# carlobaldassi/gimp-lqr-plugin

Measured on AMD Instinct MI355X. Metric: Mseams*pixels/sec on 4K RGBA, higher is better.
Workload: dtype f32; 1 GPU; batch4k: 64 x 3840x2160 RGBA per GPU, resize to 3640x2160 (200 vertical seams each), side-switch 2; images_per_gpu=64, width=3840, height=2160, new_width=3640, new_height=2160, parallelism=images sharded i mod N, no data-path collective, streams_per_gpu=1

## Files before the change

gimp-lqr-plugin_amd/csrc/lqr_shim.hip:

```cpp
#include "lqr_common.h"
#include "lqr_kernels.h"
#include "lqr_own.h"
#include <memory>

static thread_local std::string g_err;
static int g_device = -1;

static int *g_dev_err_host = nullptr;
static int *g_dev_err = nullptr;

#define HIPCK_VOID(expr) do { hipError_t e__ = (expr); if (e__ != hipSuccess) { g_err = std::string(#expr) + ": " + hipGetErrorString(e__); (void) hipGetLastError(); } } while (0)
#define HIPCK(expr)                                                                   \
    do {                                                                              \
        hipError_t e__ = (expr);                                                      \
        if (e__ != hipSuccess) {                                                      \
            g_err = std::string(#expr) + ": " + hipGetErrorString(e__);               \
            (void) hipGetLastError();                                                 \
            return (e__ == hipErrorOutOfMemory) ? LQRHIP_ENOMEM : LQRHIP_EHIP;        \
        }                                                                             \
    } while (0)

static PlanKnobs g_knobs;
static PlanDevice g_dev;

// ... 9 lines not shown
struct __attribute__((visibility("hidden"))) LqrHipCarver {
    int ch = 0;
    int depth = 0;
    int luma = 0;
    int mode = RD_RGB, alpha = -1, black = -1;
    int pix_deep = 0;
    int w0 = 0, h0 = 0;
    DevBuf<uint8_t> rgb0;
    DevBuf<int32_t> vs;
    DevBuf<float> bias0, rig0;
    int active = 0;
    int stride = 0, wk_h = 0;
    WorkingPlanes wk;
    int log_cap = 0, log_h = 0;
    int frozen_epoch = 0;
    LqrHipCarver *root = nullptr;
    std::vector<LqrHipCarver *> aux;
    LqrHipBatch *batch = nullptr;
};

static inline size_t px_bytes(const LqrHipCarver *c) { return (size_t) c->ch << (c->depth == 0 ? 0 : c->depth == 1 ? 1 : c->depth == 2 ? 2 : 3); }
static inline int32_t *vs_of(const LqrHipCarver *c) { return (c->root ? c->root : c)->vs; }

namespace {
struct PlaneJob {
    LqrHipCarver *c;
    DevBuf<uint8_t> nrgb;
    DevBuf<float> nbias, nrig;
};
}
// ... 27 lines not shown
};
static void commit(PlaneJobs &pj)
{
    for (auto &j : pj.jobs) {
        j.c->rgb0 = std::move(j.nrgb);
        if (j.nbias) j.c->bias0 = std::move(j.nbias);
        if (j.nrig) j.c->rig0 = std::move(j.nrig);
    }
}

struct PendingInflate { PlaneJobs pj; int kind = 0 , w1 = 0, h1 = 0; };

struct LqrHipBatch {
    std::vector<LqrHipCarver *> cs;
    DevCarver *d_desc = nullptr;
    hipStream_t stream = nullptr;
    DevBuf<unsigned long long> exch;
    int exch_ntiles = 0, exch_n = 0, exch_px = 0;
    int tile_epoch = 0;
    bool dirty = true;
    int shared_n = 1;
    bool shared = false;
    bool safe = false;
    std::unique_ptr<PendingInflate> pending_inflate;
};
static bool g_no_spin = false;

struct ProfRec {
    std::vector<std::pair<hipEvent_t, hipEvent_t>> ev;
    double bytes = 0;
// ... 429 lines not shown
    c->luma = luma != 0;
    return changed;
}

extern "C" int lqrhip_carver_set_read(LqrHipCarver *c, int image_type, int alpha, int black)
{
    static const int mode_of[8] = {RD_RGB, RD_RGB, RD_GREY, RD_GREY, RD_CMY, RD_CMYK, RD_CMYK, RD_CUSTOM};
    if (image_type < 0 || image_type > 7 || alpha >= c->ch || black >= c->ch) return LQRHIP_EARG;
    const bool was = reads_value(c);
    const int mode = mode_of[image_type], a = alpha < 0 ? -1 : alpha, k = black < 0 ? -1 : black;
    const bool differs = mode != c->mode || a != c->alpha || k != c->black;
    c->mode = mode; c->alpha = a; c->black = k;
    return (differs && (was || reads_value(c))) ? 1 : 0;
}

static void free_working(LqrHipCarver *c)
{
    c->wk = WorkingPlanes();
    c->log_cap = 0; c->log_h = 0;
}

extern "C" void lqrhip_carver_destroy(LqrHipCarver *c)
{
    if (!c) return;
    {
        LqrHipCarver *r = c->root ? c->root : c;
        if (r->batch && r->batch->stream) (void) hipStreamSynchronize(r->batch->stream);
        if (c->batch && c->batch != r->batch && c->batch->stream) (void) hipStreamSynchronize(c->batch->stream);
        if (g_stream0) (void) hipStreamSynchronize(g_stream0);
        (void) hipGetLastError();
    }
    delete c;
}

// ... 191 lines not shown
    tmp.done();
    return 0;
}

extern "C" void lqrhip_set_sub_batches(int n) { g_knobs.sub_batches = n > 0 ? n : 0; }
extern "C" int lqrhip_sub_batches(int n)
{
    const char *q = getenv("GPU_MAX_HW_QUEUES");
    g_dev.hw_queues = q ? atoi(q) : 0;
    return plan_streams(g_knobs, g_dev, n);
}

extern "C" void lqrhip_batch_set_shared(LqrHipBatch *b, int shared) { b->shared = shared != 0; b->shared_n = shared > 1 ? shared : 1; }
extern "C" void lqrhip_batch_set_safe(LqrHipBatch *b, int safe) { b->safe = safe != 0; if (safe) g_fault_stats[6]++; }

extern "C" LqrHipBatch *lqrhip_batch_create(LqrHipCarver **carvers, int n)
{
    if (lqrhip_init() < 0 || n <= 0) return nullptr;
    LqrHipBatch *b = new LqrHipBatch();
    for (int i = 0; i < n; i++) {
        b->cs.push_back(carvers[i]);
        carvers[i]->batch = b;
    }
    if (hipStreamCreateWithFlags(&b->stream, hipStreamNonBlocking) != hipSuccess ||
        hipMalloc((void **) &b->d_desc, sizeof(DevCarver) * n) != hipSuccess) {
        g_err = "batch_create failed";
        if (b->stream) (void) hipStreamDestroy(b->stream);
        for (auto *c : b->cs) if (c->batch == b) c->batch = nullptr;
        delete b;
        return nullptr;
    }
    g_live_batches.push_back(b);
    return b;
}

static void invalidate_all_batches(void)
{
    for (auto *b : g_live_batches) { b->exch_ntiles = 0; b->dirty = true; }
}

extern "C" void lqrhip_batch_abort(LqrHipBatch *b)
{
    if (!b) return;
    (void) hipStreamSynchronize(b->stream);
    (void) hipGetLastError();
    b->pending_inflate.reset();
    if (g_dev_err_host) *g_dev_err_host = 0;
    invalidate_all_batches();
}

extern "C" void lqrhip_batch_destroy(LqrHipBatch *b)
{
    if (!b) return;
    g_live_batches.erase(std::remove(g_live_batches.begin(), g_live_batches.end(), b), g_live_batches.end());
    if (b->stream) { (void) hipStreamSynchronize(b->stream); (void) hipStreamDestroy(b->stream); }
    for (auto *c : b->cs) if (c->batch == b) c->batch = nullptr;
    if (b->d_desc) (void) hipFree(b->d_desc);
    delete b;
}

extern "C" int lqrhip_batch_sync(LqrHipBatch *b)
{
    HIPCK(hipStreamSynchronize(b->stream));
    return check_dev_error();
}
extern "C" void *lqrhip_batch_stream(LqrHipBatch *b) { return (void *) b->stream; }

static DevCarver make_desc(const LqrHipCarver *c)
{
    DevCarver d;
    const WorkingPlanes &k = c->wk;
    d.rgb0 = c->rgb0; d.vs = vs_of(c); d.bias0 = c->bias0; d.rig0 = c->rig0;
// ... 75 lines not shown
    for (auto &e : it->second.ev) {
        float a = 0, b = 0;
        if (hipEventElapsedTime(&a, base, e.first) != hipSuccess) { (void) hipGetLastError(); float t = 0; if (hipEventElapsedTime(&t, e.first, base) == hipSuccess) a = -t; else (void) hipGetLastError(); }
        if (hipEventElapsedTime(&b, base, e.second) != hipSuccess) { (void) hipGetLastError(); float t = 0; if (hipEventElapsedTime(&t, e.second, base) == hipSuccess) b = -t; else (void) hipGetLastError(); }
        iv.emplace_back(a, b);
    }
    std::sort(iv.begin(), iv.end());
    float end = -1e30f;
    for (auto &p : iv) {
        if (p.first > end) { *ms_union += p.second - p.first; end = p.second; }
        else if (p.second > end) { *ms_union += p.second - end; end = p.second; }
    }
    return 0;
}

extern "C" int lqrhip_wk_init(LqrHipBatch *b, int from_visible)
{
    LqrHipCarver *c0 = b->cs[0];
    int w = c0->w0, h = c0->h0, rc;
    for (auto *c : b->cs) {
        if (c->w0 != w || c->h0 != h || c->ch != c0->ch || c->depth != c0->depth || c->luma != c0->luma || c->mode != c0->mode ||
            c->alpha != c0->alpha || c->black != c0->black)
            return LQRHIP_EARG;
        if ((rc = ensure_working(c, w, h))) return rc;
    }
    if ((rc = batch_upload(b))) return rc;
    for (auto *c : b->cs) c->frozen_epoch = 0;
    const dim3 grid((c0->stride + 255) / 256, h, (unsigned) b->cs.size()), grid_v(h, (unsigned) b->cs.size());
#define LAUNCH_WK(FORM, arg) do { if (from_visible) hipLaunchKernelGGL(k_wk_init_visible<FORM>, grid_v, dim3(256), 0, b->stream, b->d_desc, w, h, c0->stride, arg); \
                                  else hipLaunchKernelGGL(k_wk_init<FORM>, grid, dim3(256), 0, b->stream, b->d_desc, w, h, c0->stride, arg); } while (0)
    if (!reads_value(c0)) LAUNCH_WK(PixPacked, c0->ch);
    else if (c0->depth == 0) LAUNCH_WK(PixValue<0>, deep_read(c0));
    else if (c0->depth == 1) LAUNCH_WK(PixValue<1>, deep_read(c0));
    else if (c0->depth == 2) LAUNCH_WK(PixValue<2>, deep_read(c0));
    else LAUNCH_WK(PixValue<3>, deep_read(c0));
#undef LAUNCH_WK
    HIPCK(hipGetLastError());
    return 0;
}

extern "C" int lqrhip_emap_build(LqrHipBatch *b, const LqrHipDpParams *p, int w, int h)
{
    int rc;
    if ((rc = batch_upload(b))) return rc;
    LqrHipCarver *c0 = b->cs[0];
    dim3 grid((w + 255) / 256, h, (unsigned) b->cs.size());
    DpK k = make_dpk(p, c0->ch);
    const bool value = reads_value(c0);
    const int nrg = plane_nrg(value, nrg_index(p->nrg_func));
#define CASE(N, V) if (nrg == N && value == V) hipLaunchKernelGGL((k_emap_full<N, V>), grid, dim3(256), 0, b->stream, b->d_desc, k, w, h, c0->stride); else
    K_EMAP_FORMS(CASE) return no_form("k_emap_full");
#undef CASE
    HIPCK(hipGetLastError());
    return 0;
}

extern "C" int lqrhip_energy_out(LqrHipBatch *b, int w, int h, int transposed, int form, int depth, int image_type, void *out, int on_device)
{
// ... 187 lines not shown
{
    LqrHipCarver *c0 = b->cs[0];
    const int from = c0->frozen_epoch;
    if (to <= from) return 0;
    const int w_from = w_at_to + (to - from);
    size_t lds = (size_t) (to - from) * sizeof(int) + (size_t) w_from + 16;
    with_form(c0, [&](auto value) {
        hipLaunchKernelGGL(k_frozen_catchup<value>, dim3(h, (unsigned) b->cs.size()), dim3(256), lds, b->stream, b->d_desc, from, to, w_from, h,
                           c0->stride);
    });
    HIPCK(hipGetLastError());
    for (auto *c : b->cs) c->frozen_epoch = to;
    return 0;
}

static int launch_band_levels(LqrHipBatch *b, const DpK &k, int w, int h, int lr, int P, bool rigm)
{
    LqrHipCarver *c0 = b->cs[0];
    const size_t n = b->cs.size();
    int rc;
    const int ntiles = (w + 63) / 64;
    const size_t need_elems = 2 * ((size_t) 4 * LV_PMAX + (size_t) 2 * ntiles * 64) * n;
    if ((rc = exch_ensure(b, need_elems, ntiles, (int) n, 103))) return rc;
    const int epoch = 1 + ((b->tile_epoch++) % ((1 << 22) - 2));
    const dim3 grid((unsigned) (8 * ((n + 7) / 8) * P));
    CENSUS(LQRHIP_CENSUS_BAND_LEVELS);
    const DpForm f = dp_form(k, lr, rigm);
#define CASE(LR, RIG, DELTA, RIGM) if (f.lr == LR && f.rig == RIG && f.delta == DELTA && f.rigm == RIGM) \
        hipLaunchKernelGGL((k_band_levels<LR, RIG, DELTA, RIGM>), grid, dim3(128), 0, b->stream, b->d_desc, k, w, h, c0->stride, b->exch.get(), epoch, g_dev_err, P, (int) n); else
    K_BAND_LEVELS_FORMS(CASE) return no_form("k_band_levels");
// ... 28 lines not shown
        if (FILE *f = fopen(path, "wb")) {
            fwrite(hdr.data(), sizeof(int), hdr.size(), f); fwrite(flags.data(), sizeof(int), flags.size(), f);
            fwrite(seam.data(), sizeof(int), seam.size(), f); fwrite(m.data(), sizeof(float), np, f); fwrite(least.data(), 1, np, f);
            fclose(f);
        }
    }
    return rc;
}

static int seam_step_impl(LqrHipBatch *b, const LqrHipDpParams *p, int w, int h, int log_index, int leftright_pick,
                          int full_rebuild, int leftright_next)
{
    int rc;
    LqrHipCarver *c0 = b->cs[0];
    for (auto *c : b->cs)
        if (log_index >= c->log_cap) return LQRHIP_EARG;
    if ((rc = batch_upload(b))) return rc;
    const unsigned n = (unsigned) b->cs.size();
    DpK k = make_dpk(p, c0->ch);
    const int stride = c0->stride;
    const int wnew = w - 1;
    const int move_dp = (wnew > 1 && !full_rebuild) ? 1 : 0;
    const PlanBatch pb = plan_batch(b);
    const StepPlan s = plan_seam_step(g_knobs, g_dev, pb, p->delta_x, p->use_rigidity != 0, w, h, full_rebuild != 0, log_index + 1 - c0->frozen_epoch);
    const bool rigm = pb.rigm(p->use_rigidity != 0);
    const int moved_unit = 2 * (4 + (move_dp ? 5 : 0) + (pb.rigmask ? 4 : 0));
    if (s.backtrack == LQRHIP_CENSUS_VP_PARALLEL) {
        const int nchunks = s.vp_chunks, R4 = (s.vp_rows + 3) / 4;
        const size_t need = (size_t) (nchunks + 1) * stride + 64, need_path = need * 4 * R4;
        bool grew = false;
        for (auto *c : b->cs) {
// ... 78 lines not shown
        ProfScope ps("band_update", b->stream, 0);
        CENSUS(LQRHIP_CENSUS_BAND_GENERIC);
        hipLaunchKernelGGL(k_band_update, dim3(n), dim3(64), 0, b->stream, b->d_desc, k, wnew, h, stride, leftright_next);
    }
    {
        ProfScope ps("dp_update", b->stream, 0);
        if ((rc = launch_dp<true>(b, k, s.dp, rigm, wnew, h, leftright_next))) return rc;
    }
    HIPCK(hipGetLastError());
    return 0;
}

extern "C" int lqrhip_seam_log_reserve(LqrHipBatch *b, int n_seams, int h)
{
    int rc;
    for (auto *c : b->cs) if ((rc = ensure_log(c, n_seams, h))) return rc;
    return 0;
}

extern "C" int lqrhip_vs_commit(LqrHipBatch *b, int w0, int h0, int wc0, int n_seams, int first_level, int finish)
{
    int rc;
    if ((rc = batch_upload(b))) return rc;
    size_t lds = ((size_t) n_seams + wc0) * sizeof(int);
    if (lds > 150 * 1024) { g_err = "vs_commit: session too large for LDS"; return LQRHIP_EARG; }
    if (lds_needs_attr(lds)) {
        HIPCK(hipFuncSetAttribute((const void *) k_vs_commit, hipFuncAttributeMaxDynamicSharedMemorySize, (int) lds));
        CENSUS(LQRHIP_CENSUS_LDS_ATTR_COMMIT);
    }
    hipLaunchKernelGGL(k_vs_commit, dim3(h0, (unsigned) b->cs.size()), dim3(256), lds, b->stream, b->d_desc, w0, h0, wc0, n_seams,
                       first_level, finish);
    HIPCK(hipGetLastError());
    inject_after_commit(b, w0, h0, first_level);
    if ((rc = frozen_catchup(b, n_seams, wc0 - n_seams, h0))) return rc;
    for (auto *c : b->cs) c->frozen_epoch = 0;
    return 0;
}

static int g_selfcheck = 1, g_recovery = 1;
extern "C" void lqrhip_set_selfcheck(int on) { g_selfcheck = on != 0; }
extern "C" void lqrhip_set_recovery(int on) { g_recovery = on != 0; }
extern "C" int lqrhip_get_recovery(void) { return g_recovery; }
extern "C" int lqrhip_session_check(LqrHipBatch *b, int h, int wc0, int n_seams, int delta_x)
{
    int rc;
    if (!g_selfcheck || n_seams < 1) return 0;
    if ((rc = batch_upload(b))) return rc;
    hipLaunchKernelGGL(k_seam_check, dim3((h + 255) / 256, (unsigned) b->cs.size()), dim3(256), 0, b->stream, b->d_desc, h, wc0, n_seams, delta_x, g_dev_err);
    HIPCK(hipGetLastError());
    return 0;
}
extern "C" int lqrhip_session_rollback(LqrHipBatch *b, int w0, int h0, int first_level, int finish)
{
    (void) hipStreamSynchronize(b->stream);
    b->pending_inflate.reset();
    (void) hipGetLastError();
    if (g_dev_err_host) *g_dev_err_host = 0;
    invalidate_all_batches();
    int rc;
    if ((rc = batch_upload(b))) return rc;
    const size_t n = (size_t) w0 * h0;
    hipLaunchKernelGGL(k_vs_rollback, dim3((unsigned) std::min<size_t>((n + 255) / 256, 4096), (unsigned) b->cs.size()), dim3(256), 0, b->stream, b->d_desc, n, first_level, finish ? w0 : 0);
    HIPCK(hipGetLastError());
    HIPCK(hipStreamSynchronize(b->stream));
    for (auto *c : b->cs) c->frozen_epoch = 0;
    g_fault_stats[4]++;
    return 0;
}
static int g_inject_kind = 0, g_inject_step = 0, g_inject_times = 0;
extern "C" void lqrhip_debug_inject(int kind, int at_step, int times) { g_inject_kind = kind; g_inject_step = at_step; g_inject_times = kind ? std::max(times, 1) : 0; }
static void inject_after_step(LqrHipBatch *b, int h, int log_index)
{
    if (g_inject_times <= 0 || log_index != g_inject_step) return;
    if (g_inject_kind == 1 || g_inject_kind == 2) { *g_dev_err_host = g_inject_kind == 1 ? DEVERR_TILE_TIMEOUT : DEVERR_BAND_PREDICTION; }
    else if (g_inject_kind == 3 || g_inject_kind == 4) hipLaunchKernelGGL(k_inject, dim3(1), dim3(64), 0, b->stream, b->d_desc, g_inject_kind - 3, h, 0, log_index, 0);
    else return;
    g_inject_times--; g_fault_stats[5]++;
}
static void inject_after_commit(LqrHipBatch *b, int w0, int h0, int first_level)
{
// ... 37 lines not shown
        hipLaunchKernelGGL(k_inflate<false>, dim3(h0, (unsigned) pj.n_narrow), dim3(256), lds, b->stream, pj.d_dev.get(), w0, w1, l, max_level, g_selfcheck ? g_dev_err : (int *) nullptr);
    if (pj.n_wide())
        hipLaunchKernelGGL(k_inflate<true>, dim3(h0, (unsigned) pj.n_wide()), dim3(256), lds, b->stream, pj.d_wide(), w0, w1, l, max_level, g_selfcheck ? g_dev_err : (int *) nullptr);
    HIPCK(hipGetLastError());
    HIPCK(hipStreamSynchronize(b->stream));
    if ((rc = check_dev_error())) return rc;
    return st.kept();
}
extern "C" int lqrhip_planes_commit(LqrHipBatch *b)
{
    PendingInflate *pi = b->pending_inflate.get();
    if (!pi) return LQRHIP_EARG;
    PlaneJobs &pj = pi->pj;
    commit(pj);
    for (auto &j : pj.jobs) { j.c->w0 = pi->w1; j.c->h0 = pi->h1; }
    if (pi->kind != 2) {
        size_t i = 0;
        for (auto *c : b->cs) c->vs = std::move(pj.new_vs[i++]);
    }
    b->dirty = true;
    b->pending_inflate.reset();
    return 0;
}
extern "C" int lqrhip_inflate_commit(LqrHipBatch *b) { return lqrhip_planes_commit(b); }

extern "C" int lqrhip_flatten(LqrHipBatch *b, int w0, int h0, int w, int level)
{
    int rc;
    Staging st(b, 1, w, h0);
    PlaneJobs &pj = st.jobs();
// ... 85 lines not shown
    HIPCK(hipMemsetAsync(dout, 0, sizeof(int), g_stream0));
    hipLaunchKernelGGL(k_mask_line_max, dim3(n_lines), dim3(256), 0, g_stream0, d, channels, width, a0, b0, line_len, direction, dout);
    HIPCK(hipGetLastError());
    HIPCK(hipMemcpyAsync(&result, dout, sizeof(int), hipMemcpyDeviceToHost, g_stream0));
    HIPCK(hipStreamSynchronize(g_stream0));
    tmp.done();
    return result;
}

extern "C" void lqrhip_pool_trim(void)
{
    (void) hipDeviceSynchronize();
    for (auto &kv : g_pool_free) { (void) hipFree(kv.second); g_pool_size.erase(kv.second); }
    g_pool_free.clear();
    g_pool_cached = 0;
}

extern "C" int lqrhip_device_sync(void)
{
    HIPCK(hipDeviceSynchronize());
    return check_dev_error();
}

extern "C" int lqrhip_read_vmap(LqrHipCarver *c, int w0, int h0, int w, int level, int depth, int *out)
{
    int rc = batch_sync_of(c);
    if (rc) return rc;
    size_t n = (size_t) w * h0;
    Scratch tmp(g_stream0);
    int32_t *d = tmp.get<int32_t>(n, "&d", rc);
// ... 23 lines not shown
        for (int y = 0; y < h; y++) memcpy(en + (size_t) y * w, t.data() + (size_t) y * c->stride + org, (size_t) w * sizeof(float));
    }
    if (m) {
        HIPCK(hipMemcpy(t.data(), c->wk.m, n * sizeof(float), hipMemcpyDeviceToHost));
        for (int y = 0; y < h; y++) memcpy(m + (size_t) y * w, t.data() + (size_t) y * c->stride + org, (size_t) w * sizeof(float));
    }
    if (least_dx) {
        HIPCK(hipMemcpy(tl.data(), c->wk.least, n, hipMemcpyDeviceToHost));
        for (int y = 0; y < h; y++)
            for (int x = 0; x < w; x++) least_dx[(size_t) y * w + x] = y == 0 ? 0 : (int) tl[(size_t) y * c->stride + org + x];
    }
    return 0;
}

__global__ __launch_bounds__(256) void k_copy16(const u32x4 *__restrict__ src, u32x4 *__restrict__ dst, size_t n16);
extern "C" int lqrhip_carver_reset(LqrHipCarver *c, const void *device_rgb, int w, int h)
{
    if (!c || c->root || !c->aux.empty() || w < 1 || h < 1) return LQRHIP_EARG;
    int rc = batch_sync_of(c);
    if (rc) return rc;
    const size_t n = (size_t) w * h;
    c->rgb0.reset(); c->vs.reset(); c->bias0.reset(); c->rig0.reset();
    if (c->wk.bias || c->wk.rig) { free_working(c); c->stride = 0; c->wk_h = 0; }
    c->w0 = w; c->h0 = h;
    c->frozen_epoch = 0;
    if ((rc = c->rgb0.alloc(n * px_bytes(c), "&c->rgb0")) || (rc = c->vs.alloc(n, "&c->vs"))) return rc;
    {
        const size_t bytes = n * px_bytes(c), n16 = bytes / 16;
        if (n16 && !(((uintptr_t) device_rgb | (uintptr_t) c->rgb0.get()) & 15)) {
            hipLaunchKernelGGL(k_copy16, dim3((unsigned) ((n16 + 255) / 256)), dim3(256), 0, g_stream0, (const u32x4 *) device_rgb, (u32x4 *) c->rgb0.get(), n16);
            HIPCK(hipGetLastError());
            if (bytes & 15) HIPCK(hipMemcpyAsync(c->rgb0 + n16 * 16, (const uint8_t *) device_rgb + n16 * 16, bytes & 15, hipMemcpyDeviceToDevice, g_stream0));
        } else {
            HIPCK(hipMemcpyAsync(c->rgb0, device_rgb, bytes, hipMemcpyDeviceToDevice, g_stream0));
        }
    }
    HIPCK(hipMemsetAsync(c->vs, 0, n * sizeof(int32_t), g_stream0));
    if (c->batch) c->batch->dirty = true;
    if (c->active && (rc = ensure_working(c, w, h))) return rc;
    return 0;
}

extern "C" int lqrhip_reset_sync(void)
{
    if (g_stream0) HIPCK(hipStreamSynchronize(g_stream0));
    return 0;
}

extern "C" int lqrhip_mem_info(unsigned long long *free_bytes, unsigned long long *total_bytes, unsigned long long *cached_bytes)
{
    if (lqrhip_init() < 0) return LQRHIP_EHIP;
    size_t f = 0, t = 0;
    HIPCK(hipMemGetInfo(&f, &t));
    if (free_bytes) *free_bytes = f;
    if (total_bytes) *total_bytes = t;
    if (cached_bytes) *cached_bytes = g_pool_cached;
    return 0;
}

__global__ __launch_bounds__(256) void k_copy16(const u32x4 *__restrict__ src, u32x4 *__restrict__ dst, size_t n16)
{
    const size_t i = (size_t) blockIdx.x * 256 + threadIdx.x;
    if (i < n16) __builtin_nontemporal_store(__builtin_nontemporal_load((const GLOBAL_AS u32x4 *) src + i), (GLOBAL_AS u32x4 *) dst + i);
}

extern "C" int lqrhip_copy_bandwidth(unsigned long long bytes, int iters, double *gbps)
{
    if (lqrhip_init() < 0) return LQRHIP_EHIP;
    if (iters < 1 || bytes < 4096) return LQRHIP_EARG;
    struct Event { hipEvent_t e = nullptr; ~Event() { if (e) (void) hipEventDestroy(e); } } e0, e1;
    int rc;
    Scratch tmp(g_stream0);
    uint8_t *a = tmp.get<uint8_t>(bytes, "&a", rc);
    if (rc) return rc;
    uint8_t *b = tmp.get<uint8_t>(bytes, "&b", rc);
    if (rc) return rc;
    float ms = 0;
    const size_t n16 = bytes / 16;
// ... 57 lines not shown
```

gimp-lqr-plugin_amd/host/lqr_carver.c:

```c
#include <stdlib.h>
#include <string.h>
#include <stdio.h>
#include <math.h>

#include "../../include/lqr.h"
#include "../../include/lqr_coldepth.h"
#include "../../include/lqr_imagetype.h"
#include "../../include/lqr_masks.h"
#include "../../include/lqr_energy.h"
#include "../../include/lqr_hip.h"
#include "lqr_mask_queue.h"

#define MAXI(a, b) ((a) > (b) ? (a) : (b))
#define MINI(a, b) ((a) < (b) ? (a) : (b))

struct _LqrProgress {
    gfloat update_step;
    LqrProgressFuncInit init;
    LqrProgressFuncUpdate update;
    LqrProgressFuncEnd end;
    gchar init_width_message[LQR_PROGRESS_MAX_MESSAGE_LENGTH];
    gchar end_width_message[LQR_PROGRESS_MAX_MESSAGE_LENGTH];
    gchar init_height_message[LQR_PROGRESS_MAX_MESSAGE_LENGTH];
    gchar end_height_message[LQR_PROGRESS_MAX_MESSAGE_LENGTH];
};

struct _LqrVMap {
    gint *buffer;
    gint width, height, depth, orientation;
// ... 655 lines not shown
        if (w_before - 1 > 1) {
            if (r0->lr_switch_frequency && ((l - r0->max_level + lr_switch_interval / 2) % lr_switch_interval) == 0) {
                for (i = 0; i < g->n; i++) g->r[i]->leftright ^= 1;
                full = 1;
            }
        } else {
            finish = 1;
        }
        HIP_ALL(g, lqrhip_seam_step(B, &p, w_before, r0->h, l - r0->max_level, lr_pick, full, r0->leftright));
        for (i = 0; i < g->n; i++) { g->r[i]->level++; g->r[i]->w--; }
    }

    if (g_debug_snapshot)
        for (i = 0; i < g->n; i++) LQR_CATCH(take_debug_snapshot(g->r[i]));

    HIP_ALL(g, lqrhip_session_check(B, r0->h, wc0, n_seams, r0->delta_x));
    HIP_ALL(g, lqrhip_batch_sync(B));
    HIP_ALL(g, lqrhip_vs_commit(B, r0->w0, r0->h0, wc0, n_seams, first_level, finish));
    HIP_ALL(g, lqrhip_inflate(B, r0->w0, r0->h0, depth - 1, r0->max_level));
    HIP_ALL(g, lqrhip_planes_commit(B));
    w1 = r0->w0 + (depth - 1) - r0->max_level + 1;
    FOR_TREE(g, i, r, {
        r->level = depth; r->max_level = depth;
        r->w0 = w1;
        set_width_one(r, r->w_start);
    });
    return LQR_OK;
}

static LqrRetVal session_run(Group *g, int depth, int redo, int *reported)
{
    LqrCarver *r0 = g->r[0];
    LqrHipDpParams p;
    int i;
    for (i = 0; i < g->n; i++) set_width_one(g->r[i], g->r[i]->w_start - g->r[i]->max_level + 1);
// ... 168 lines not shown
static LqrRetVal group_resize(LqrCarver **rs, int n, int w1, int h1)
{
    Group g;
    LqrRetVal ret = LQR_OK;
    int i;
    if (w1 < 1 || h1 < 1) return LQR_ERROR;
    for (i = 0; i < n; i++)
        if (rs[i]->root || !rs[i]->progress) return LQR_ERROR;
    for (i = 0; i < n; i++) LQR_CATCH(mask_queue_flush(rs[i]));
    for (i = 0; i < n; i++)
        if (frame_refused(rs[i], w1, 0) || frame_refused(rs[i], h1, 1)) {
            fprintf(stderr, "liblqr-hip: resize refused: a frame wider than %d px in the direction being carved is not supported\n",
                    LQRHIP_MAX_FRAME_WIDTH);
            return LQR_ERROR;
        }
    LQR_CATCH(group_open(&g, rs, n));
    if (rs[0]->resize_order == LQR_RES_ORDER_HOR) {
        if ((ret = group_resize_dir(&g, w1, 0)) == LQR_OK) ret = group_resize_dir(&g, h1, 1);
    } else {
        if ((ret = group_resize_dir(&g, h1, 1)) == LQR_OK) ret = group_resize_dir(&g, w1, 0);
    }
    if (ret == LQR_OK) {
        int k;
        for (k = 0; k < g.nb; k++) { LqrRetVal rk = hip_ret(lqrhip_batch_sync(g.b[k])); if (ret == LQR_OK) ret = rk; }
    }
    if (ret != LQR_OK) { int k; for (k = 0; k < g.nb; k++) lqrhip_batch_abort(g.b[k]); }
    FOR_TREE(&g, i, r, { r->ro_valid = 0; r->ro_line = 0; r->ro_x = 0; });
    group_close(&g);
    return ret;
}

LqrRetVal lqr_carver_resize(LqrCarver *r, gint w1, gint h1) { return group_resize(&r, 1, w1, h1); }

LqrRetVal lqrx_carver_resize_batch(LqrCarver **carvers, gint n, gint w1, gint h1)
{
    int i, same = 1;
    if (n < 1) return LQR_ERROR;
    for (i = 1; i < n; i++) same &= same_config(carvers[0], carvers[i]);
    if (same) {
        const LqrCarver *c = carvers[0];
        if (is_general(c)) {
            int wmax = c->w_start > c->h_start ? c->w_start : c->h_start, lim;
            if (w1 > wmax) wmax = w1;
// ... 102 lines not shown
LqrRetVal lqrx_carver_read_image_device(LqrCarver *r, void *device_ptr)
{
    HIP_CATCH(lqrhip_read_visible_device(r->dev, r->w0, r->h0, r->w, r->level, device_ptr));
    return LQR_OK;
}

LqrRetVal lqrx_vmap_to_rgba(LqrVMap *v, const gdouble col_start[3], const gdouble col_end[3], guchar *out_rgba)
{
    if (!v || !v->buffer || !out_rgba) return LQR_ERROR;
    HIP_CATCH(lqrhip_vmap_to_rgba(v->buffer, v->width, v->height, v->depth, col_start, col_end, out_rgba));
    return LQR_OK;
}

LqrRetVal lqrx_carver_reload_device_batch(LqrCarver **rs, gint n, void *const *device_rgb)
{
    int i, x;
    if (n < 1) return LQR_ERROR;
    for (i = 0; i < n; i++)
        if (!rs[i] || rs[i]->root || rs[i]->attached || !device_rgb[i]) return LQR_ERROR;
    for (i = 0; i < n; i++) {
        LqrCarver *r = rs[i];
        LqrVMapList *v, *vn;
        lqr_maskq_reset(&r->mq[0]); lqr_maskq_reset(&r->mq[1]);
        HIP_CATCH(lqrhip_carver_reset(r->dev, device_rgb[i], r->img_w, r->img_h));
        for (v = r->flushed_vs; v; v = vn) { vn = v->next; lqr_vmap_destroy(v->current); free(v); }
        r->flushed_vs = NULL;
        r->level = r->max_level = 1;
        r->w = r->w0 = r->w_start = r->img_w;
        r->h = r->h0 = r->h_start = r->img_h;
        r->transposed = 0;
        r->leftright = 0;
        r->has_bias = r->has_rigmask = 0;
        r->wk_valid = 0;
        r->ro_valid = 0; r->ro_line = 0; r->ro_x = 0;
        if (r->active)
            for (x = -r->delta_x; x <= r->delta_x; x++)
                r->rigidity_map[x + r->delta_x] = r->rigidity * powf(fabsf((float) x), 1.5f) / r->h;
    }
    HIP_CATCH(lqrhip_reset_sync());
    return LQR_OK;
}

gint lqrx_guess_new_size(const guchar *mask, gint channels, gint width, gint height, gint x_off, gint y_off,
                         gint old_width, gint old_height, gint direction)
{
    int lw = MINI(old_width, width + x_off) - MAXI(0, x_off);
    int lh = MINI(old_height, height + y_off) - MAXI(0, y_off);
    int old_size = direction ? old_height : old_width, m;
    if (direction == 0)
        m = lqrhip_mask_line_max(mask, channels, width, height, MAXI(0, y_off) - y_off, MAXI(0, -x_off),
                                 MINI(old_height, height + y_off) - MAXI(0, y_off), lw, 0);
    else
        m = lqrhip_mask_line_max(mask, channels, width, height, MAXI(0, x_off) - x_off, MAXI(0, -y_off),
                                 MINI(old_width, width + x_off) - MAXI(0, x_off), lh, 1);
// ... 82 lines not shown
```

include/lqr_hip.h:

```cpp
#ifndef LQR_HIP_H
#define LQR_HIP_H

#include <stddef.h>

#ifdef __cplusplus
extern "C" {
#endif

#define LQRHIP_OK 0
#define LQRHIP_ENOMEM (-2)
#define LQRHIP_EHIP (-1)
#define LQRHIP_EARG (-3)
#define LQRHIP_EFAULT (-4)
#define LQRHIP_MAX_DELTA 16
#define LQRHIP_MAX_CHANNELS 64
#define LQRHIP_MAX_FRAME_WIDTH 16384

typedef struct LqrHipCarver LqrHipCarver;
typedef struct LqrHipBatch LqrHipBatch;

typedef struct LqrHipDpParams {
    int delta_x;
    int use_rigidity;
    float rigidity_map[2 * LQRHIP_MAX_DELTA + 1];
    int nrg_func;
    int nrg_radius;
    int w_start;
} LqrHipDpParams;

int lqrhip_init(void);
const char *lqrhip_last_error(void);

LqrHipCarver *lqrhip_carver_create(const unsigned char *rgb, int w, int h, int channels);
LqrHipCarver *lqrhip_carver_create_ext(const void *rgb, int w, int h, int channels, int depth);
int lqrhip_carver_set_read_luma(LqrHipCarver *c, int luma);
int lqrhip_carver_set_read(LqrHipCarver *c, int image_type, int alpha, int black);
void lqrhip_carver_destroy(LqrHipCarver *c);
int lqrhip_carver_reset(LqrHipCarver *c, const void *device_rgb, int w, int h);
int lqrhip_reset_sync(void);
int lqrhip_carver_attach(LqrHipCarver *root, LqrHipCarver *aux);
int lqrhip_carver_activate(LqrHipCarver *c);

int lqrhip_mask_add(LqrHipCarver *c, const unsigned char *mask, int channels, int width, int height,
                    int x_off, int y_off, int transposed, int is_rigmask, int bias_factor);

int lqrhip_mask_add_f(LqrHipCarver *c, const void *mask, int depth, int on_device, int width, int height, int x_off, int y_off,
                      int transposed, int is_rigmask, int bias_factor);
int lqrhip_mask_plane_ensure(LqrHipCarver *c, int is_rigmask);
int lqrhip_mask_scatter(LqrHipCarver *c, int is_rigmask, const int *index, const double *value, const size_t *start, int buckets);
int lqrhip_mask_clear(LqrHipCarver *c, int is_rigmask);
int lqrhip_read_mask_plane(LqrHipCarver *c, int is_rigmask, int transposed, float *out);
unsigned long long lqrhip_debug_mask_flushes(void);

// ... 16 lines not shown
                     int leftright_pick, int full_rebuild, int leftright_next);
int lqrhip_seam_log_reserve(LqrHipBatch *b, int n_seams, int h);
int lqrhip_vs_commit(LqrHipBatch *b, int w0, int h0, int wc0, int n_seams, int first_level, int finish);
int lqrhip_session_check(LqrHipBatch *b, int h, int wc0, int n_seams, int delta_x);
void lqrhip_set_selfcheck(int on);
void lqrhip_set_recovery(int on);
int lqrhip_get_recovery(void);
int lqrhip_session_rollback(LqrHipBatch *b, int w0, int h0, int first_level, int finish);
void lqrhip_batch_set_safe(LqrHipBatch *b, int safe);
void lqrhip_set_no_spin(int on);
int lqrhip_get_no_spin(void);
int lqrhip_fault_stats(unsigned long long *out8, int reset);
void lqrhip_debug_inject(int kind, int at_step, int times);
void lqrhip_debug_fail_alloc(int nth);
unsigned long long lqrhip_debug_pool_live(void);
int lqrhip_inflate(LqrHipBatch *b, int w0, int h0, int l, int max_level);
int lqrhip_flatten(LqrHipBatch *b, int w0, int h0, int w, int level);
int lqrhip_transpose(LqrHipBatch *b, int w, int h);
int lqrhip_planes_commit(LqrHipBatch *b);
int lqrhip_inflate_commit(LqrHipBatch *b);

int lqrhip_read_visible(LqrHipCarver *c, int w0, int h0, int w, int level, unsigned char *out);
int lqrhip_mask_line_max(const unsigned char *mask, int channels, int width, int height, int a0, int b0, int n_lines, int line_len,
                         int direction);
int lqrhip_read_visible_device(LqrHipCarver *c, int w0, int h0, int w, int level, void *device_out);
int lqrhip_device_sync(void);
int lqrhip_mem_info(unsigned long long *free_bytes, unsigned long long *total_bytes, unsigned long long *cached_bytes);
int lqrhip_copy_bandwidth(unsigned long long bytes, int iters, double *gbps);
int lqrhip_vmap_to_rgba(const int *vmap, int w, int h, int depth, const double col_start[3], const double col_end[3],
                        unsigned char *out_rgba);
// ... 47 lines not shown
```

Baseline: 501,300 Mseams*px/s.

## Cut fixed per-call costs: park streams, batch resets, defer frozen catchup

Destroyed batches now park their streams and descriptor buffers in a small pool for reuse instead of recreating them with hipStreamCreate and hipMalloc. Carver resets for a batch of same-sized images are merged into one multi-job kernel that copies the RGB planes and zeroes the seam maps, replacing a memcpy and memset per image. The frozen-epoch catchup after vs_commit is deferred and paid lazily at the next emap build or log reserve, so it can be skipped when state is dropped anyway. Optional host timing instrumentation is added behind a compile flag. This adds state-tracking complexity around deferred catchup and pooled resources.

```diff
diff --git a/gimp-lqr-plugin_amd/csrc/lqr_shim.hip b/gimp-lqr-plugin_amd/csrc/lqr_shim.hip
--- a/gimp-lqr-plugin_amd/csrc/lqr_shim.hip
+++ b/gimp-lqr-plugin_amd/csrc/lqr_shim.hip
@@ -47,6 +47,7 @@
     WorkingPlanes wk;
     int log_cap = 0, log_h = 0;
     int frozen_epoch = 0;
+    int owed_to = 0, owed_w = 0, owed_h = 0;
     LqrHipCarver *root = nullptr;
     std::vector<LqrHipCarver *> aux;
     LqrHipBatch *batch = nullptr;
@@ -104,6 +105,7 @@
 struct LqrHipBatch {
     std::vector<LqrHipCarver *> cs;
     DevCarver *d_desc = nullptr;
+    size_t desc_cap = 0;
     hipStream_t stream = nullptr;
     DevBuf<unsigned long long> exch;
     int exch_ntiles = 0, exch_n = 0, exch_px = 0;
@@ -563,10 +565,17 @@
     return (differs && (was || reads_value(c))) ? 1 : 0;
 }
 
+static inline void drop_catchup(LqrHipCarver *c)
+{
+    c->owed_to = 0; c->owed_w = 0; c->owed_h = 0;
+    c->frozen_epoch = 0;
+}
+
 static void free_working(LqrHipCarver *c)
 {
     c->wk = WorkingPlanes();
     c->log_cap = 0; c->log_h = 0;
+    drop_catchup(c);
 }
 
 extern "C" void lqrhip_carver_destroy(LqrHipCarver *c)
@@ -788,6 +797,24 @@
 extern "C" void lqrhip_batch_set_shared(LqrHipBatch *b, int shared) { b->shared = shared != 0; b->shared_n = shared > 1 ? shared : 1; }
 extern "C" void lqrhip_batch_set_safe(LqrHipBatch *b, int safe) { b->safe = safe != 0; if (safe) g_fault_stats[6]++; }
 
+static const size_t MAX_PARKED = 4;
+static std::vector<hipStream_t> g_parked_streams;
+static unsigned long long g_fixed_stats[3];
+static std::multimap<size_t, DevCarver *> g_parked_desc;
+extern "C" void lqrhip_debug_fixedcost(unsigned long long out4[4], int reset)
+{
+    out4[0] = g_parked_streams.size();
+    for (int i = 0; i < 3; i++) out4[i + 1] = g_fixed_stats[i];
+    if (reset) memset(g_fixed_stats, 0, sizeof g_fixed_stats);
+}
+static void unpark_all(void)
+{
+    for (hipStream_t s : g_parked_streams) (void) hipStreamDestroy(s);
+    g_parked_streams.clear();
+    for (auto &kv : g_parked_desc) (void) hipFree(kv.second);
+    g_parked_desc.clear();
+}
+
 extern "C" LqrHipBatch *lqrhip_batch_create(LqrHipCarver **carvers, int n)
 {
     if (lqrhip_init() < 0 || n <= 0) return nullptr;
@@ -796,9 +823,17 @@
         b->cs.push_back(carvers[i]);
         carvers[i]->batch = b;
     }
-    if (hipStreamCreateWithFlags(&b->stream, hipStreamNonBlocking) != hipSuccess ||
-        hipMalloc((void **) &b->d_desc, sizeof(DevCarver) * n) != hipSuccess) {
+    hipError_t e = hipSuccess;
+    if (!g_parked_streams.empty()) { b->stream = g_parked_streams.back(); g_parked_streams.pop_back(); g_fixed_stats[0]++; }
+    else e = hipStreamCreateWithFlags(&b->stream, hipStreamNonBlocking);
+    if (e == hipSuccess) {
+        auto it = g_parked_desc.lower_bound((size_t) n);
+        if (it != g_parked_desc.end()) { b->d_desc = it->second; b->desc_cap = it->first; g_parked_desc.erase(it); }
+        else if ((e = hipMalloc((void **) &b->d_desc, sizeof(DevCarver) * n)) == hipSuccess) b->desc_cap = (size_t) n;
+    }
+    if (e != hipSuccess) {
         g_err = "batch_create failed";
+        (void) hipGetLastError();
         if (b->stream) (void) hipStreamDestroy(b->stream);
         for (auto *c : b->cs) if (c->batch == b) c->batch = nullptr;
         delete b;
@@ -827,9 +862,16 @@
 {
     if (!b) return;
     g_live_batches.erase(std::remove(g_live_batches.begin(), g_live_batches.end(), b), g_live_batches.end());
-    if (b->stream) { (void) hipStreamSynchronize(b->stream); (void) hipStreamDestroy(b->stream); }
+    if (b->stream) (void) hipStreamSynchronize(b->stream);
     for (auto *c : b->cs) if (c->batch == b) c->batch = nullptr;
-    if (b->d_desc) (void) hipFree(b->d_desc);
+    if (b->stream) {
+        if (g_parked_streams.size() < MAX_PARKED) g_parked_streams.push_back(b->stream);
+        else (void) hipStreamDestroy(b->stream);
+    }
+    if (b->d_desc) {
+        if (g_parked_desc.size() < MAX_PARKED) g_parked_desc.emplace(b->desc_cap, b->d_desc);
+        else (void) hipFree(b->d_desc);
+    }
     delete b;
 }
 
@@ -935,6 +977,7 @@
     return 0;
 }
 
+static int pay_catchup(LqrHipBatch *b);
 extern "C" int lqrhip_wk_init(LqrHipBatch *b, int from_visible)
 {
     LqrHipCarver *c0 = b->cs[0];
@@ -946,7 +989,7 @@
         if ((rc = ensure_working(c, w, h))) return rc;
     }
     if ((rc = batch_upload(b))) return rc;
-    for (auto *c : b->cs) c->frozen_epoch = 0;
+    for (auto *c : b->cs) drop_catchup(c);
     const dim3 grid((c0->stride + 255) / 256, h, (unsigned) b->cs.size()), grid_v(h, (unsigned) b->cs.size());
 #define LAUNCH_WK(FORM, arg) do { if (from_visible) hipLaunchKernelGGL(k_wk_init_visible<FORM>, grid_v, dim3(256), 0, b->stream, b->d_desc, w, h, c0->stride, arg); \
                                   else hipLaunchKernelGGL(k_wk_init<FORM>, grid, dim3(256), 0, b->stream, b->d_desc, w, h, c0->stride, arg); } while (0)
@@ -963,6 +1006,7 @@
 extern "C" int lqrhip_emap_build(LqrHipBatch *b, const LqrHipDpParams *p, int w, int h)
 {
     int rc;
+    if ((rc = pay_catchup(b))) return rc;
     if ((rc = batch_upload(b))) return rc;
     LqrHipCarver *c0 = b->cs[0];
     dim3 grid((w + 255) / 256, h, (unsigned) b->cs.size());
@@ -1180,6 +1224,36 @@
     return 0;
 }
 
+static int pay_catchup(LqrHipBatch *b)
+{
+    LqrHipCarver *c0 = b->cs[0];
+    bool any = false, alike = true;
+    for (auto *c : b->cs) {
+        any |= c->owed_to > 0;
+        alike &= c->owed_to == c0->owed_to && c->owed_w == c0->owed_w && c->owed_h == c0->owed_h && c->frozen_epoch == c0->frozen_epoch && c->stride == c0->stride;
+    }
+    if (!any) return 0;
+    int rc;
+    if ((rc = batch_upload(b))) return rc;
+    if (alike) {
+        if ((rc = frozen_catchup(b, c0->owed_to, c0->owed_w, c0->owed_h))) return rc;
+    } else {
+        for (size_t i = 0; i < b->cs.size(); i++) {
+            LqrHipCarver *c = b->cs[i];
+            if (c->owed_to <= c->frozen_epoch) continue;
+            const int from = c->frozen_epoch, w_from = c->owed_w + (c->owed_to - from);
+            const size_t lds = (size_t) (c->owed_to - from) * sizeof(int) + (size_t) w_from + 16;
+            with_form(c, [&](auto value) {
+                hipLaunchKernelGGL(k_frozen_catchup<value>, dim3(c->owed_h, 1), dim3(256), lds, b->stream, b->d_desc + i, from, c->owed_to, w_from, c->owed_h, c->stride);
+            });
+            HIPCK(hipGetLastError());
+            drop_catchup(c);
+        }
+    }
+    for (auto *c : b->cs) drop_catchup(c);
+    return 0;
+}
+
 static int launch_band_levels(LqrHipBatch *b, const DpK &k, int w, int h, int lr, int P, bool rigm)
 {
     LqrHipCarver *c0 = b->cs[0];
@@ -1238,7 +1312,7 @@
     int rc;
     LqrHipCarver *c0 = b->cs[0];
     for (auto *c : b->cs)
-        if (log_index >= c->log_cap) return LQRHIP_EARG;
+        if (log_index >= c->log_cap || c->owed_to) return LQRHIP_EARG;
     if ((rc = batch_upload(b))) return rc;
     const unsigned n = (unsigned) b->cs.size();
     DpK k = make_dpk(p, c0->ch);
@@ -1347,6 +1421,7 @@
 extern "C" int lqrhip_seam_log_reserve(LqrHipBatch *b, int n_seams, int h)
 {
     int rc;
+    if ((rc = pay_catchup(b))) return rc;
     for (auto *c : b->cs) if ((rc = ensure_log(c, n_seams, h))) return rc;
     return 0;
 }
@@ -1365,8 +1440,10 @@
                        first_level, finish);
     HIPCK(hipGetLastError());
     inject_after_commit(b, w0, h0, first_level);
-    if ((rc = frozen_catchup(b, n_seams, wc0 - n_seams, h0))) return rc;
-    for (auto *c : b->cs) c->frozen_epoch = 0;
+    for (auto *c : b->cs) {
+        if (c->frozen_epoch < n_seams) { c->owed_to = n_seams; c->owed_w = wc0 - n_seams; c->owed_h = h0; }
+        else drop_catchup(c);
+    }
     return 0;
 }
 
@@ -1396,7 +1473,7 @@
     hipLaunchKernelGGL(k_vs_rollback, dim3((unsigned) std::min<size_t>((n + 255) / 256, 4096), (unsigned) b->cs.size()), dim3(256), 0, b->stream, b->d_desc, n, first_level, finish ? w0 : 0);
     HIPCK(hipGetLastError());
     HIPCK(hipStreamSynchronize(b->stream));
-    for (auto *c : b->cs) c->frozen_epoch = 0;
+    for (auto *c : b->cs) drop_catchup(c);
     g_fault_stats[4]++;
     return 0;
 }
@@ -1464,6 +1541,8 @@
     PlaneJobs &pj = pi->pj;
     commit(pj);
     for (auto &j : pj.jobs) { j.c->w0 = pi->w1; j.c->h0 = pi->h1; }
+    if (pi->kind != 0)
+        for (auto *c : b->cs) drop_catchup(c);
     if (pi->kind != 2) {
         size_t i = 0;
         for (auto *c : b->cs) c->vs = std::move(pj.new_vs[i++]);
@@ -1579,6 +1658,7 @@
     for (auto &kv : g_pool_free) { (void) hipFree(kv.second); g_pool_size.erase(kv.second); }
     g_pool_free.clear();
     g_pool_cached = 0;
+    unpark_all();
 }
 
 extern "C" int lqrhip_device_sync(void)
@@ -1632,17 +1712,24 @@
 }
 
 __global__ __launch_bounds__(256) void k_copy16(const u32x4 *__restrict__ src, u32x4 *__restrict__ dst, size_t n16);
-extern "C" int lqrhip_carver_reset(LqrHipCarver *c, const void *device_rgb, int w, int h)
-{
-    if (!c || c->root || !c->aux.empty() || w < 1 || h < 1) return LQRHIP_EARG;
+static int reset_planes(LqrHipCarver *c, int w, int h)
+{
     int rc = batch_sync_of(c);
     if (rc) return rc;
     const size_t n = (size_t) w * h;
     c->rgb0.reset(); c->vs.reset(); c->bias0.reset(); c->rig0.reset();
     if (c->wk.bias || c->wk.rig) { free_working(c); c->stride = 0; c->wk_h = 0; }
     c->w0 = w; c->h0 = h;
-    c->frozen_epoch = 0;
+    drop_catchup(c);
     if ((rc = c->rgb0.alloc(n * px_bytes(c), "&c->rgb0")) || (rc = c->vs.alloc(n, "&c->vs"))) return rc;
+    return 0;
+}
+extern "C" int lqrhip_carver_reset(LqrHipCarver *c, const void *device_rgb, int w, int h)
+{
+    if (!c || c->root || !c->aux.empty() || w < 1 || h < 1) return LQRHIP_EARG;
+    int rc = reset_planes(c, w, h);
+    if (rc) return rc;
+    const size_t n = (size_t) w * h;
     {
         const size_t bytes = n * px_bytes(c), n16 = bytes / 16;
         if (n16 && !(((uintptr_t) device_rgb | (uintptr_t) c->rgb0.get()) & 15)) {
@@ -1659,6 +1746,56 @@
     return 0;
 }
 
+enum { RESET_JOBS = 16 };
+struct ResetJob { const uint8_t *src; uint8_t *dst; uint8_t *vs; size_t bytes; };
+struct ResetJobs { ResetJob j[RESET_JOBS]; };
+__global__ __launch_bounds__(256) void k_reset_jobs(const ResetJobs jobs, const size_t vs_bytes);
+static int g_reset_batch_count = 0;
+extern "C" int lqrhip_carver_reset_batch_count(void) { return g_reset_batch_count; }
+extern "C" int lqrhip_carver_reset_batch(LqrHipCarver **cs, const void *const *device_rgb, int n, int w, int h)
+{
+    g_reset_batch_count = 0;
+    if (!cs || !device_rgb || n < 1 || w < 1 || h < 1) return LQRHIP_EARG;
+    for (int i = 0; i < n; i++)
+        if (!cs[i] || cs[i]->root || !cs[i]->aux.empty() || !device_rgb[i]) return LQRHIP_EARG;
+    const size_t npx = (size_t) w * h, vs_bytes = npx * sizeof(int32_t);
+    ResetJobs jobs = {};
+    int nj = 0;
+    size_t most = vs_bytes;
+    auto flush = [&]() -> int {
+        if (!nj) return 0;
+        const unsigned blocks = (unsigned) std::min<size_t>((most / 16 + 255) / 256 + 1, 4096);
+        hipLaunchKernelGGL(k_reset_jobs, dim3(blocks, (unsigned) nj), dim3(256), 0, g_stream0, jobs, vs_bytes);
+        nj = 0; most = vs_bytes;
+        HIPCK(hipGetLastError());
+        return 0;
+    };
+    for (int i = 0; i < n; i++) {
+        LqrHipCarver *c = cs[i];
+        g_reset_batch_count = i;
+        int rc = reset_planes(c, w, h);
+        if (rc) { (void) flush(); return rc; }
+        const size_t bytes = npx * px_bytes(c);
+        if (!(((uintptr_t) device_rgb[i] | (uintptr_t) c->rgb0.get() | (uintptr_t) c->vs.get()) & 15)) {
+            jobs.j[nj++] = ResetJob{(const uint8_t *) device_rgb[i], c->rgb0.get(), (uint8_t *) c->vs.get(), bytes};
+            most = std::max(most, bytes);
+            g_fixed_stats[1]++;
+        } else {
+            g_fixed_stats[2]++;
+            hipError_t e = hipMemcpyAsync(c->rgb0, device_rgb[i], bytes, hipMemcpyDeviceToDevice, g_stream0);
+            if (e == hipSuccess) e = hipMemsetAsync(c->vs, 0, vs_bytes, g_stream0);
+            if (e != hipSuccess) { (void) flush(); HIPCK(e); }
+        }
+        if (c->batch) c->batch->dirty = true;
+        if (c->active && (rc = ensure_working(c, w, h))) { (void) flush(); return rc; }
+        if (nj == RESET_JOBS && (rc = flush())) return rc;
+    }
+    int rc = flush();
+    if (rc) return rc;
+    g_reset_batch_count = n;
+    return 0;
+}
+
 extern "C" int lqrhip_reset_sync(void)
 {
     if (g_stream0) HIPCK(hipStreamSynchronize(g_stream0));
@@ -1680,6 +1817,20 @@
 {
     const size_t i = (size_t) blockIdx.x * 256 + threadIdx.x;
     if (i < n16) __builtin_nontemporal_store(__builtin_nontemporal_load((const GLOBAL_AS u32x4 *) src + i), (GLOBAL_AS u32x4 *) dst + i);
+}
+
+__global__ __launch_bounds__(256) void k_reset_jobs(const ResetJobs jobs, const size_t vs_bytes)
+{
+    const ResetJob j = jobs.j[blockIdx.y];
+    const size_t tid = (size_t) blockIdx.x * 256 + threadIdx.x, nthreads = (size_t) gridDim.x * 256;
+    const size_t n16 = j.bytes / 16, z16 = vs_bytes / 16;
+    for (size_t i = tid; i < n16; i += nthreads)
+        __builtin_nontemporal_store(__builtin_nontemporal_load((const GLOBAL_AS u32x4 *) j.src + i), (GLOBAL_AS u32x4 *) j.dst + i);
+    const u32x4 zero = {0u, 0u, 0u, 0u};
+    for (size_t i = tid; i < z16; i += nthreads) __builtin_nontemporal_store(zero, (GLOBAL_AS u32x4 *) j.vs + i);
+    const size_t back = nthreads - 1 - tid;
+    if (back < (j.bytes & 15)) j.dst[n16 * 16 + back] = j.src[n16 * 16 + back];
+    if (back < (vs_bytes & 15)) j.vs[z16 * 16 + back] = 0;
 }
 
 extern "C" int lqrhip_copy_bandwidth(unsigned long long bytes, int iters, double *gbps)
diff --git a/gimp-lqr-plugin_amd/host/lqr_carver.c b/gimp-lqr-plugin_amd/host/lqr_carver.c
--- a/gimp-lqr-plugin_amd/host/lqr_carver.c
+++ b/gimp-lqr-plugin_amd/host/lqr_carver.c
@@ -1,3 +1,6 @@
+#ifdef LQRHIP_TIMING
+#define _POSIX_C_SOURCE 199309L
+#endif
 #include <stdlib.h>
 #include <string.h>
 #include <stdio.h>
@@ -13,6 +16,26 @@
 
 #define MAXI(a, b) ((a) > (b) ? (a) : (b))
 #define MINI(a, b) ((a) < (b) ? (a) : (b))
+
+#ifdef LQRHIP_TIMING
+#include <time.h>
+enum { T_RELOAD, T_OPEN, T_CLOSE, T_TAIL, T_PARTS };
+static double g_t_sum[T_PARTS];
+static long g_t_calls[T_PARTS];
+static double t_now(void) { struct timespec ts; clock_gettime(CLOCK_MONOTONIC, &ts); return ts.tv_sec * 1e3 + ts.tv_nsec * 1e-6; }
+__attribute__((destructor)) static void t_report(void)
+{
+    static const char *const name[T_PARTS] = {"reload", "group_open", "group_close", "session_tail"};
+    int i;
+    for (i = 0; i < T_PARTS; i++)
+        if (g_t_calls[i]) fprintf(stderr, "LQRHIP_TIMING %s calls %ld total_ms %.3f mean_ms %.4f\n", name[i], g_t_calls[i], g_t_sum[i], g_t_sum[i] / g_t_calls[i]);
+}
+#define T_BEGIN(part) const double t_begin_##part = t_now()
+#define T_END(part) do { g_t_sum[part] += t_now() - t_begin_##part; g_t_calls[part]++; } while (0)
+#else
+#define T_BEGIN(part) do { } while (0)
+#define T_END(part) do { } while (0)
+#endif
 
 struct _LqrProgress {
     gfloat update_step;
@@ -698,11 +721,13 @@
     if (g_debug_snapshot)
         for (i = 0; i < g->n; i++) LQR_CATCH(take_debug_snapshot(g->r[i]));
 
+    T_BEGIN(T_TAIL);
     HIP_ALL(g, lqrhip_session_check(B, r0->h, wc0, n_seams, r0->delta_x));
     HIP_ALL(g, lqrhip_batch_sync(B));
     HIP_ALL(g, lqrhip_vs_commit(B, r0->w0, r0->h0, wc0, n_seams, first_level, finish));
     HIP_ALL(g, lqrhip_inflate(B, r0->w0, r0->h0, depth - 1, r0->max_level));
     HIP_ALL(g, lqrhip_planes_commit(B));
+    T_END(T_TAIL);
     w1 = r0->w0 + (depth - 1) - r0->max_level + 1;
     FOR_TREE(g, i, r, {
         r->level = depth; r->max_level = depth;
@@ -901,7 +926,11 @@
                     LQRHIP_MAX_FRAME_WIDTH);
             return LQR_ERROR;
         }
-    LQR_CATCH(group_open(&g, rs, n));
+    {
+        T_BEGIN(T_OPEN);
+        LQR_CATCH(group_open(&g, rs, n));
+        T_END(T_OPEN);
+    }
     if (rs[0]->resize_order == LQR_RES_ORDER_HOR) {
         if ((ret = group_resize_dir(&g, w1, 0)) == LQR_OK) ret = group_resize_dir(&g, h1, 1);
     } else {
@@ -913,7 +942,11 @@
     }
     if (ret != LQR_OK) { int k; for (k = 0; k < g.nb; k++) lqrhip_batch_abort(g.b[k]); }
     FOR_TREE(&g, i, r, { r->ro_valid = 0; r->ro_line = 0; r->ro_x = 0; });
-    group_close(&g);
+    {
+        T_BEGIN(T_CLOSE);
+        group_close(&g);
+        T_END(T_CLOSE);
+    }
     return ret;
 }
 
@@ -1046,15 +1079,25 @@
 
 LqrRetVal lqrx_carver_reload_device_batch(LqrCarver **rs, gint n, void *const *device_rgb)
 {
-    int i, x;
+    int i, x, lo, rc = 0, done = 0;
+    LqrHipCarver **ds;
+    T_BEGIN(T_RELOAD);
     if (n < 1) return LQR_ERROR;
     for (i = 0; i < n; i++)
         if (!rs[i] || rs[i]->root || rs[i]->attached || !device_rgb[i]) return LQR_ERROR;
-    for (i = 0; i < n; i++) {
+    ds = (LqrHipCarver **) malloc((size_t) n * sizeof *ds);
+    if (!ds) return LQR_NOMEM;
+    for (i = 0; i < n; i++) ds[i] = rs[i]->dev;
+    for (lo = 0; lo < n && !rc; lo = i) {
+        for (i = lo + 1; i < n && rs[i]->img_w == rs[lo]->img_w && rs[i]->img_h == rs[lo]->img_h; i++);
+        rc = lqrhip_carver_reset_batch(ds + lo, (const void *const *) device_rgb + lo, i - lo, rs[lo]->img_w, rs[lo]->img_h);
+        done = rc ? lo + lqrhip_carver_reset_batch_count() : i;
+    }
+    free(ds);
+    for (i = 0; i < done; i++) {
         LqrCarver *r = rs[i];
         LqrVMapList *v, *vn;
         lqr_maskq_reset(&r->mq[0]); lqr_maskq_reset(&r->mq[1]);
-        HIP_CATCH(lqrhip_carver_reset(r->dev, device_rgb[i], r->img_w, r->img_h));
         for (v = r->flushed_vs; v; v = vn) { vn = v->next; lqr_vmap_destroy(v->current); free(v); }
         r->flushed_vs = NULL;
         r->level = r->max_level = 1;
@@ -1069,7 +1112,9 @@
             for (x = -r->delta_x; x <= r->delta_x; x++)
                 r->rigidity_map[x + r->delta_x] = r->rigidity * powf(fabsf((float) x), 1.5f) / r->h;
     }
+    HIP_CATCH(rc);
     HIP_CATCH(lqrhip_reset_sync());
+    T_END(T_RELOAD);
     return LQR_OK;
 }
 
diff --git a/include/lqr_hip.h b/include/lqr_hip.h
--- a/include/lqr_hip.h
+++ b/include/lqr_hip.h
@@ -37,6 +37,8 @@
 int lqrhip_carver_set_read(LqrHipCarver *c, int image_type, int alpha, int black);
 void lqrhip_carver_destroy(LqrHipCarver *c);
 int lqrhip_carver_reset(LqrHipCarver *c, const void *device_rgb, int w, int h);
+int lqrhip_carver_reset_batch(LqrHipCarver **cs, const void *const *device_rgb, int n, int w, int h);
+int lqrhip_carver_reset_batch_count(void);
 int lqrhip_reset_sync(void);
 int lqrhip_carver_attach(LqrHipCarver *root, LqrHipCarver *aux);
 int lqrhip_carver_activate(LqrHipCarver *c);
@@ -83,6 +85,7 @@
 void lqrhip_debug_inject(int kind, int at_step, int times);
 void lqrhip_debug_fail_alloc(int nth);
 unsigned long long lqrhip_debug_pool_live(void);
+void lqrhip_debug_fixedcost(unsigned long long out4[4], int reset);
 int lqrhip_inflate(LqrHipBatch *b, int w0, int h0, int l, int max_level);
 int lqrhip_flatten(LqrHipBatch *b, int w0, int h0, int w, int level);
 int lqrhip_transpose(LqrHipBatch *b, int w, int h);
```

Result: faster. 506,600 Mseams*px/s (median of 6 runs) (+1.1%).
